# zc402/video-classification

Measured on AMD Instinct MI355X. Metric: clips/sec SlowFast-R50 8x8, 32x224^2 bf16 training step, higher is better.
Workload: dtype bf16

## Files before the change

video-classification_amd/csrc/conv_pw.hip:

```cpp
#include "sfk_common.h"

namespace {

struct PwK {
  const void* x;
  void* y;
  const void* w;
  const void* res;
  const float *scale, *shift, *rscale, *rshift;
  uint8_t* bits;
  const uint8_t* mbits;
  float* parts;
  int xld, xoff, yld, yoff, rld, roff;
  int M, K, cout, relu;
  uint32_t xbytes, ybytes, rbytes;
};

__device__ __forceinline__ int slab_off(int r, int s) { return r * 64 + ((s ^ ((4 - ((r >> 2) & 3)) & 3)) << 4); }

__device__ __forceinline__ void swap16f(float& a, float& b) {
  const auto r = __builtin_amdgcn_permlane16_swap(__float_as_uint(a), __float_as_uint(b), false, false);
  a = __uint_as_float(r[0]);
  b = __uint_as_float(r[1]);
}

template <int NF, int KS, int CG, int NT, bool XDB, int MODE = 0>
__global__ __launch_bounds__(NT, 2) void conv_pw_fused_kernel(const PwK k) {
  constexpr bool DG = MODE == 1;
  constexpr int CW = NF * 16;
  extern __shared__ __attribute__((aligned(16))) char smem[];
  char* wl = smem;
  float* coef = reinterpret_cast<float*>(smem + KS * k.cout * 64);
  const int tid = threadIdx.x, lane = tid & 63, wave = tid >> 6;
  const int l15 = lane & 15, g = lane >> 4;
  {
    const __amdgpu_buffer_rsrc_t wrs = sfk_make_rsrc(k.w, (uint32_t)k.cout * (uint32_t)k.K * 2u);
    const int segs = k.cout * KS * 4;
    for (int i = tid; i < segs; i += NT) {
      const int s = i & 3, ks = (i >> 2) % KS, r = i / (4 * KS);
      const int kk = ks * 32 + s * 8;
      const uint4 v = sfk_buffer_load16(wrs, kk < k.K ? (uint32_t)((r * k.K + kk) * 2) : SFK_OOB);
      *reinterpret_cast<uint4*>(wl + ks * k.cout * 64 + slab_off(r, s)) = v;
    }
    if (MODE == 0) for (int i = tid; i < k.cout; i += NT) {
      coef[i] = k.scale ? k.scale[i] : 1.f;
      coef[k.cout + i] = (k.shift ? k.shift[i] : 0.f) + ((k.res && k.rshift) ? k.rshift[i] : 0.f);
      coef[2 * k.cout + i] = (k.res && k.rscale) ? k.rscale[i] : 1.f;
    }
  }
  __syncthreads();

  const __amdgpu_buffer_rsrc_t xrs = sfk_make_rsrc(k.x, k.xbytes);
  const __amdgpu_buffer_rsrc_t rrs = sfk_make_rsrc(k.res, k.res ? k.rbytes : 0u);
  const bool has_res = k.res != nullptr;
  constexpr int WPB = NT / 64;
  const int wg = (blockIdx.x * WPB + wave);
  const int cgi = wg % CG, wi = wg / CG, nw = (gridDim.x * WPB) / CG;
  const int co_w = cgi * CW;
  const int ntiles = (k.M + 15) >> 4;
  const bf16_t* __restrict__ dummy = nullptr;
  (void)dummy;

  uint4 xc[KS], xn[XDB ? KS : 1];
  uint4 rc[NF / 2], rn[NF / 2];
  uint32_t mc[DG ? NF / 2 : 1], mn[DG ? NF / 2 : 1];
  float csum[DG ? NF / 2 : 1][8];
  if constexpr (DG) {
#pragma unroll
    for (int p = 0; p < NF / 2; ++p)
#pragma unroll
      for (int e = 0; e < 8; ++e) csum[p][e] = 0.f;
  }
  auto issue_x = [&](int tile, uint4 (&xv)[KS]) __attribute__((always_inline)) {
    int m = tile * 16 + l15;
    if (m >= k.M) m = k.M - 1;
    const uint32_t xrow = (uint32_t)(((int64_t)m * k.xld + k.xoff) * 2);
#pragma unroll
    for (int ks = 0; ks < KS; ++ks) {
      const int kk = ks * 32 + g * 8;
      xv[ks] = sfk_buffer_load16(xrs, kk < k.K ? xrow + (uint32_t)(kk * 2) : SFK_OOB);
    }
  };
  auto issue_r = [&](int tile, uint4 (&rv)[NF / 2], uint32_t (&mv)[DG ? NF / 2 : 1]) __attribute__((always_inline)) {
    if (has_res) {
      int m = tile * 16 + l15;
      if (m >= k.M) m = k.M - 1;
      const uint32_t rrow = (uint32_t)(((int64_t)m * k.rld + k.roff + co_w) * 2);
#pragma unroll
      for (int p = 0; p < NF / 2; ++p)
        rv[p] = sfk_buffer_load16(rrs, rrow + (uint32_t)((32 * p + 16 * (g & 1) + 8 * (g >> 1)) * 2));
      if constexpr (DG) {
#pragma unroll
        for (int p = 0; p < NF / 2; ++p)
          mv[p] = k.mbits[(int64_t)m * (k.cout >> 3) + ((co_w + 32 * p + 16 * (g & 1) + 8 * (g >> 1)) >> 3)];
      }
    }
  };

  int tile = wi;
  if (MODE == 0 && tile >= ntiles) return;
  if (tile < ntiles) {
    issue_x(tile, xc);
    issue_r(tile, rc, mc);
  }
  bf16_t* __restrict__ yp = static_cast<bf16_t*>(k.y);
  for (; tile < ntiles; tile += nw) {
    const int nxt = tile + nw;
    if (nxt < ntiles) {
      if constexpr (XDB) issue_x(nxt, reinterpret_cast<uint4(&)[KS]>(xn));
      issue_r(nxt, rn, mn);
    }
    f32x4 acc[NF];
#pragma unroll
    for (int i = 0; i < NF; ++i) acc[i] = f32x4{0.f, 0.f, 0.f, 0.f};
    const char* wlt = wl;
    if constexpr (NF * KS >= 32) asm volatile("" : "+v"(wlt));
#pragma unroll
    for (int ks = 0; ks < KS; ++ks) {
      const bf16x8 b = __builtin_bit_cast(bf16x8, xc[ks]);
#pragma unroll
      for (int i = 0; i < NF; ++i) {
        const bf16x8 a = *reinterpret_cast<const bf16x8*>(wlt + ks * k.cout * 64 + slab_off(co_w + 16 * i + l15, g));
        acc[i] = __builtin_amdgcn_mfma_f32_16x16x32_bf16(a, b, acc[i], 0, 0, 0);
      }
    }
    if constexpr (!XDB) {
      if (nxt < ntiles) issue_x(nxt, xc);
    }
    const int m = tile * 16 + l15;
    const bool rok = m < k.M;
    const int64_t yrow = (int64_t)m * k.yld + k.yoff;
#pragma unroll
    for (int p = 0; p < NF / 2; ++p) {
      float v[8] = {acc[2 * p][0], acc[2 * p][1], acc[2 * p][2], acc[2 * p][3],
                    acc[2 * p + 1][0], acc[2 * p + 1][1], acc[2 * p + 1][2], acc[2 * p + 1][3]};
#pragma unroll
      for (int e = 0; e < 4; ++e) swap16f(v[e], v[4 + e]);
      const int co = co_w + 32 * p + 16 * (g & 1) + 8 * (g >> 1);
      if constexpr (DG) {
        const bf16x8 r8 = __builtin_bit_cast(bf16x8, rc[p]);
        bf16x8 o;
#pragma unroll
        for (int e = 0; e < 8; ++e) {
          const float f = ((mc[p] >> e) & 1u) ? v[e] + (float)r8[e] : 0.f;
          o[e] = (bf16_t)f;
          if (rok) csum[p][e] += (float)o[e];
        }
        if (rok) *reinterpret_cast<bf16x8*>(yp + yrow + co) = o;
        continue;
      }
      const float4 s0 = *reinterpret_cast<const float4*>(coef + co), s1 = *reinterpret_cast<const float4*>(coef + co + 4);
      const float4 h0 = *reinterpret_cast<const float4*>(coef + k.cout + co), h1 = *reinterpret_cast<const float4*>(coef + k.cout + co + 4);
      const float sc[8] = {s0.x, s0.y, s0.z, s0.w, s1.x, s1.y, s1.z, s1.w};
      const float sh[8] = {h0.x, h0.y, h0.z, h0.w, h1.x, h1.y, h1.z, h1.w};
      float f[8];
#pragma unroll
      for (int e = 0; e < 8; ++e) f[e] = v[e] * sc[e] + sh[e];
      if (has_res) {
        const float4 q0 = *reinterpret_cast<const float4*>(coef + 2 * k.cout + co), q1 = *reinterpret_cast<const float4*>(coef + 2 * k.cout + co + 4);
        const float rs[8] = {q0.x, q0.y, q0.z, q0.w, q1.x, q1.y, q1.z, q1.w};
        const bf16x8 r8 = __builtin_bit_cast(bf16x8, rc[p]);
#pragma unroll
        for (int e = 0; e < 8; ++e) f[e] += (float)r8[e] * rs[e];
      }
      uint32_t bits = 0;
      bf16x8 o;
#pragma unroll
      for (int e = 0; e < 8; ++e) {
        if (k.relu) {
          bits |= (f[e] > 0.f ? 1u : 0u) << e;
          f[e] = f[e] > 0.f ? f[e] : 0.f;
        }
        o[e] = (bf16_t)f[e];
      }
      if (rok) {
        *reinterpret_cast<bf16x8*>(yp + yrow + co) = o;
        if (k.bits) k.bits[(int64_t)m * (k.cout >> 3) + (co >> 3)] = (uint8_t)bits;
      }
    }
    if constexpr (XDB) {
#pragma unroll
      for (int ks = 0; ks < KS; ++ks) xc[ks] = xn[ks];
    }
#pragma unroll
    for (int p = 0; p < NF / 2; ++p) rc[p] = rn[p];
    if constexpr (DG) {
#pragma unroll
      for (int p = 0; p < NF / 2; ++p) mc[p] = mn[p];
    }
  }
  if constexpr (DG) {
    float* row = k.parts + (int64_t)wi * k.cout * 2;
#pragma unroll
    for (int p = 0; p < NF / 2; ++p) {
#pragma unroll
      for (int e = 0; e < 8; ++e) {
        float t = csum[p][e];
#pragma unroll
        for (int sft = 1; sft < 16; sft <<= 1) t += __shfl_xor(t, sft);
        csum[p][e] = t;
      }
      if (l15 == 0) {
        const int co = co_w + 32 * p + 16 * (g & 1) + 8 * (g >> 1);
#pragma unroll
        for (int e = 0; e < 8; ++e) *reinterpret_cast<float2*>(row + (co + e) * 2) = make_float2(csum[p][e], 0.f);
      }
    }
  }
}

inline int pw_blocks(int M, int CG, int NT) {
  const int WPB = NT / 64;
  const int ntiles = (M + 15) / 16;
  int blocks = 256 * (NT == 512 ? 1 : 2);
  while ((blocks * WPB) % CG) --blocks;
  int need = (ntiles * CG + WPB - 1) / WPB;
  while ((need * WPB) % CG) ++need;
  return blocks < need ? blocks : need;
}

template <int NF, int KS, int CG, int NT, bool XDB, int MODE = 0>
int pw_launch(const PwK& k, hipStream_t s, int* dry, int kernel) {
  if (dry) {
    *dry = SFK_IGEMM_ROUTE(kernel, 1, 32 * KS, NF * 16 * CG, MODE, 0, 1);
    return SFK_OK;
  }
  const size_t lds = (size_t)KS * k.cout * 64 + (size_t)3 * k.cout * 4;
  static bool attr_set = false;
  if (lds > 64 * 1024 && !attr_set) {
    if (hipFuncSetAttribute(reinterpret_cast<const void*>(&conv_pw_fused_kernel<NF, KS, CG, NT, XDB, MODE>),
                            hipFuncAttributeMaxDynamicSharedMemorySize, (int)lds) != hipSuccess)
      return SFK_ERR_LAUNCH;
    attr_set = true;
  }
  hipLaunchKernelGGL((conv_pw_fused_kernel<NF, KS, CG, NT, XDB, MODE>), dim3(pw_blocks(k.M, CG, NT)), dim3(NT), lds, s, k);
  SFK_CHECK_LAUNCH();
  return SFK_OK;
}

typedef __bf16 bf16x2_t __attribute__((ext_vector_type(2)));

template <int C1, int C2, int CO>
__global__ __launch_bounds__(256, 4) void pw_dual_kernel(const bf16_t* __restrict__ x1, int ld1, int off1,
                                                      const bf16_t* __restrict__ x2, int ld2, int off2,
                                                      const bf16_t* __restrict__ w1, const bf16_t* __restrict__ w2,
                                                      const float* __restrict__ bias, bf16_t* __restrict__ y, int ldy, int offy,
                                                      int64_t pixels) {
  constexpr int KP = (C1 + C2) / 2;
  __shared__ __attribute__((aligned(16))) uint32_t wl[CO * KP];
  __shared__ float bl[CO];
  for (int i = threadIdx.x; i < CO * KP; i += 256) {
    const int co = i / KP, kp = i % KP;
    const bf16_t* src = kp < C1 / 2 ? w1 + co * C1 + 2 * kp : w2 + co * C2 + 2 * (kp - C1 / 2);
    wl[i] = *reinterpret_cast<const uint32_t*>(src);
  }
  if (threadIdx.x < CO) bl[threadIdx.x] = bias ? bias[threadIdx.x] : 0.f;
  __syncthreads();
  constexpr int U = 1;
  for (int64_t p0 = (int64_t)blockIdx.x * 256 * U + threadIdx.x; p0 < pixels; p0 += (int64_t)gridDim.x * 256 * U) {
    uint4 a[U][C1 / 8], b[U][C2 / 8];
#pragma unroll
    for (int u = 0; u < U; ++u) {
      const int64_t p = p0 + u * 256 < pixels ? p0 + u * 256 : p0;
#pragma unroll
      for (int i = 0; i < C1 / 8; ++i) a[u][i] = *reinterpret_cast<const uint4*>(x1 + p * ld1 + off1 + 8 * i);
#pragma unroll
      for (int i = 0; i < C2 / 8; ++i) b[u][i] = *reinterpret_cast<const uint4*>(x2 + p * ld2 + off2 + 8 * i);
    }
    uint32_t woff = 0;
    for (int c8 = 0; c8 < CO; c8 += 8) {
      float acc[U][8];
#pragma unroll
      for (int j = 0; j < 8; ++j) {
        const int co = c8 + j;
#pragma unroll
        for (int u = 0; u < U; ++u) acc[u][j] = bl[co];
#pragma unroll
        for (int q = 0; q < KP / 4; ++q) {
          const uint4 wv = *reinterpret_cast<const uint4*>(&wl[co * KP + 4 * q + woff]);
          const uint32_t wp[4] = {wv.x, wv.y, wv.z, wv.w};
#pragma unroll
          for (int u = 0; u < U; ++u) {
            const uint4 xv = q < C1 / 8 ? a[u][q < C1 / 8 ? q : 0] : b[u][q >= C1 / 8 ? q - C1 / 8 : 0];
            const uint32_t xp[4] = {xv.x, xv.y, xv.z, xv.w};
#pragma unroll
            for (int e = 0; e < 4; ++e)
              acc[u][j] = __builtin_amdgcn_fdot2_f32_bf16(__builtin_bit_cast(bf16x2_t, xp[e]), __builtin_bit_cast(bf16x2_t, wp[e]),
                                                          acc[u][j], false);
          }
        }
        asm volatile("" : "+v"(woff) : "v"(acc[0][j]));
      }
#pragma unroll
      for (int u = 0; u < U; ++u) {
        const int64_t p = p0 + u * 256;
        if (p < pixels) {
          bf16x8 o;
#pragma unroll
          for (int e = 0; e < 8; ++e) o[e] = (bf16_t)acc[u][e];
          *reinterpret_cast<bf16x8*>(y + p * ldy + offy + c8) = o;
        }
      }
    }
  }
}

inline bool pw_dual_map_ok(const sfk_fmap* f) {
  return sfk_fmap_ok(f) && f->dtype == SFK_BF16 && (f->c % 8) == 0 && (f->ld % 8) == 0 && (f->c_off % 8) == 0 &&
         (((uintptr_t)f->ptr) & 15) == 0;
}

}

int sfk_conv_pw_fused(const sfk_conv_desc* d, hipStream_t s, int* dry, int kernel) {
  const sfk_conv_epilogue& e = d->ep;
  const int K = d->cin, C = d->cout;
  if (K > 128 || (K % 8) != 0) return SFK_ERR_UNSUPPORTED;
  if (sfk_fmap_bytes(&d->y) >= (1ll << 32) - 64 || sfk_fmap_bytes(&d->x) >= (1ll << 32) - 64) return SFK_ERR_UNSUPPORTED;
  const int KS = (K + 31) / 32;
  PwK k;
  k.x = d->x.ptr; k.y = d->y.ptr; k.w = d->w; k.res = e.res.ptr;
  k.scale = e.scale; k.shift = e.shift; k.rscale = e.res_scale; k.rshift = e.res_shift;
  k.bits = e.relu_bits; k.mbits = nullptr; k.parts = nullptr;
  k.xld = d->x.ld; k.xoff = d->x.c_off; k.yld = d->y.ld; k.yoff = d->y.c_off;
  k.rld = e.res.ptr ? e.res.ld : 0; k.roff = e.res.ptr ? e.res.c_off : 0;
  k.M = (int)sfk_fmap_pixels(&d->y); k.K = K; k.cout = C; k.relu = e.relu;
  k.xbytes = (uint32_t)sfk_fmap_bytes(&d->x); k.ybytes = (uint32_t)sfk_fmap_bytes(&d->y);
  k.rbytes = e.res.ptr ? (uint32_t)sfk_fmap_bytes(&e.res) : 0u;
  if (d->accumulate) {
    if (k.res) return SFK_ERR_UNSUPPORTED;
    k.res = d->y.ptr; k.rld = d->y.ld; k.roff = d->y.c_off; k.rbytes = k.ybytes;
  }
  if (C == 64 && KS == 2) return pw_launch<4, 2, 1, 256, true>(k, s, dry, kernel);
  if (C == 128 && KS == 4) return pw_launch<8, 4, 1, 256, true>(k, s, dry, kernel);
  if (C == 32 && KS == 1) return pw_launch<2, 1, 1, 256, true>(k, s, dry, kernel);
  if (C == 64 && KS == 1) return pw_launch<4, 1, 1, 256, true>(k, s, dry, kernel);
  if (C == 128 && KS == 1) return pw_launch<8, 1, 1, 256, true>(k, s, dry, kernel);
  if (C == 256 && KS == 2) return sfk_tune().igemm_pw_stream == 2 ? pw_launch<4, 2, 4, 256, true>(k, s, dry, kernel) : pw_launch<8, 2, 2, 256, true>(k, s, dry, kernel);
  if (C == 512 && KS == 4) return pw_launch<4, 4, 8, 512, true>(k, s, dry, kernel);
  if (C == 320 && KS == 4 && !k.res) return pw_launch<4, 4, 5, 512, true>(k, s, dry, kernel);
  return SFK_ERR_UNSUPPORTED;
}

int sfk_conv_pw_dgrad_rows(const sfk_conv_desc* d) {
  if (sfk_fmap_bytes(&d->y) >= (1ll << 32) - 64 || sfk_fmap_bytes(&d->x) >= (1ll << 32) - 64) return 0;
  const int M = (int)sfk_fmap_pixels(&d->y);
  if (d->cin == 64 && d->cout == 256) return pw_blocks(M, 2, 256) * 4 / 2;
  if (d->cin == 128 && d->cout == 512) return pw_blocks(M, 8, 512) * 8 / 8;
  return 0;
}

int sfk_conv_pw_dgrad(const sfk_conv_desc* d, hipStream_t s, int* dry) {
  PwK k;
  k.x = d->x.ptr; k.y = d->y.ptr; k.w = d->w; k.res = d->y.ptr;
  k.scale = k.shift = k.rscale = k.rshift = nullptr;
  k.bits = nullptr; k.mbits = d->out_relu_bits; k.parts = d->bnb.partials;
  k.xld = d->x.ld; k.xoff = d->x.c_off; k.yld = d->y.ld; k.yoff = d->y.c_off; k.rld = d->y.ld; k.roff = d->y.c_off;
  k.M = (int)sfk_fmap_pixels(&d->y); k.K = d->cin; k.cout = d->cout; k.relu = 0;
  k.xbytes = (uint32_t)sfk_fmap_bytes(&d->x); k.ybytes = (uint32_t)sfk_fmap_bytes(&d->y); k.rbytes = k.ybytes;
  if (d->cin == 64 && d->cout == 256) return pw_launch<8, 2, 2, 256, true, 1>(k, s, dry, SFK_IK_PWD);
  if (d->cin == 128 && d->cout == 512) return pw_launch<4, 4, 8, 512, true, 1>(k, s, dry, SFK_IK_PWD);
  return SFK_ERR_UNSUPPORTED;
}

extern "C" int sfk_conv_pw_dual_supported(const sfk_fmap* x1, const sfk_fmap* x2, const sfk_fmap* y) {
  if (!x1 || !x2 || !y || !pw_dual_map_ok(x1) || !pw_dual_map_ok(x2) || !pw_dual_map_ok(y)) return 0;
  if (sfk_fmap_pixels(x1) != sfk_fmap_pixels(y) || sfk_fmap_pixels(x2) != sfk_fmap_pixels(y)) return 0;
  return (x1->c == 32 && x2->c == 8 && y->c == 8) || (x1->c == 64 && x2->c == 16 && y->c == 16);
}

extern "C" int sfk_conv_pw_dual(const sfk_fmap* x1, const void* w1, const sfk_fmap* x2, const void* w2, const float* bias,
                                const sfk_fmap* y, sfk_stream_t stream) {
  if (!x1 || !x2 || !y || !w1 || !w2 || !sfk_fmap_ok(x1) || !sfk_fmap_ok(x2) || !sfk_fmap_ok(y)) return SFK_ERR_INVALID;
  if (!sfk_conv_pw_dual_supported(x1, x2, y)) return SFK_ERR_UNSUPPORTED;
  if ((((uintptr_t)w1) | ((uintptr_t)w2)) & 3) return SFK_ERR_INVALID;
  const int64_t px = sfk_fmap_pixels(y);
  int64_t blocks = (px + 255) / 256;
  if (blocks > 4096) blocks = 4096;
  hipStream_t s = static_cast<hipStream_t>(stream);
  const bf16_t *a = static_cast<const bf16_t*>(x1->ptr), *b = static_cast<const bf16_t*>(x2->ptr);
  const bf16_t *u = static_cast<const bf16_t*>(w1), *v = static_cast<const bf16_t*>(w2);
  bf16_t* o = static_cast<bf16_t*>(y->ptr);
  if (y->c == 8)
    hipLaunchKernelGGL((pw_dual_kernel<32, 8, 8>), dim3((unsigned)blocks), dim3(256), 0, s, a, x1->ld, x1->c_off, b, x2->ld, x2->c_off,
                       u, v, bias, o, y->ld, y->c_off, px);
  else
    hipLaunchKernelGGL((pw_dual_kernel<64, 16, 16>), dim3((unsigned)blocks), dim3(256), 0, s, a, x1->ld, x1->c_off, b, x2->ld, x2->c_off,
                       u, v, bias, o, y->ld, y->c_off, px);
  SFK_CHECK_LAUNCH();
  return SFK_OK;
}
```

Measured before the change: 1176.

## Add wide pointwise conv kernel with deeper prefetch for 512/320-channel outputs

Adds a new pointwise-conv forward kernel for the C=512 and C=320 (K=128) cases. Each wave computes a wider strip of output channels, NF=8 or 10 instead of 4, reading filter fragments from LDS per tile rather than keeping them in registers. It also keeps two tiles of input and residual loads in flight ahead of compute. The aim is to cut redundant activation reads across channel groups and to hide global-load latency. The cost is higher register pressure and repeated LDS filter reads. The old path stays reachable through a tuning flag bit.

```diff
diff --git a/video-classification_amd/csrc/conv_pw.hip b/video-classification_amd/csrc/conv_pw.hip
--- a/video-classification_amd/csrc/conv_pw.hip
+++ b/video-classification_amd/csrc/conv_pw.hip
@@ -209,6 +209,136 @@
   }
 }
 
+template <int NF, int KS>
+__device__ __forceinline__ void pw_wide_tile(const PwK& k, const char* wl, const float* coef, const int tile, const int co_w,
+                                             const int l15, const int g, const bool has_res, const uint4 (&xc)[KS],
+                                             const uint4 (&rc)[NF / 2]) {
+  f32x4 acc[NF];
+#pragma unroll
+  for (int i = 0; i < NF; ++i) acc[i] = f32x4{0.f, 0.f, 0.f, 0.f};
+  int wo = 0;
+  asm volatile("" : "+v"(wo));
+  const char* wlt = wl + wo;
+#pragma unroll
+  for (int ks = 0; ks < KS; ++ks) {
+    const bf16x8 b = __builtin_bit_cast(bf16x8, xc[ks]);
+#pragma unroll
+    for (int i = 0; i < NF; ++i) {
+      const bf16x8 a = *reinterpret_cast<const bf16x8*>(wlt + ks * k.cout * 64 + slab_off(co_w + 16 * i + l15, g));
+      acc[i] = __builtin_amdgcn_mfma_f32_16x16x32_bf16(a, b, acc[i], 0, 0, 0);
+    }
+  }
+  bf16_t* __restrict__ yp = static_cast<bf16_t*>(k.y);
+  const int m = tile * 16 + l15;
+  const bool rok = m < k.M;
+  const int64_t yrow = (int64_t)m * k.yld + k.yoff;
+#pragma unroll
+  for (int p = 0; p < NF / 2; ++p) {
+    float v[8] = {acc[2 * p][0], acc[2 * p][1], acc[2 * p][2], acc[2 * p][3],
+                  acc[2 * p + 1][0], acc[2 * p + 1][1], acc[2 * p + 1][2], acc[2 * p + 1][3]};
+#pragma unroll
+    for (int e = 0; e < 4; ++e) swap16f(v[e], v[4 + e]);
+    const int co = co_w + 32 * p + 16 * (g & 1) + 8 * (g >> 1);
+    const float4 s0 = *reinterpret_cast<const float4*>(coef + co), s1 = *reinterpret_cast<const float4*>(coef + co + 4);
+    const float4 h0 = *reinterpret_cast<const float4*>(coef + k.cout + co), h1 = *reinterpret_cast<const float4*>(coef + k.cout + co + 4);
+    const float sc[8] = {s0.x, s0.y, s0.z, s0.w, s1.x, s1.y, s1.z, s1.w};
+    const float sh[8] = {h0.x, h0.y, h0.z, h0.w, h1.x, h1.y, h1.z, h1.w};
+    float f[8];
+#pragma unroll
+    for (int e = 0; e < 8; ++e) f[e] = v[e] * sc[e] + sh[e];
+    uint4 rr = rc[p];
+    asm volatile("" : "+v"(rr.x), "+v"(rr.y), "+v"(rr.z), "+v"(rr.w));
+    if (has_res) {
+      const float4 q0 = *reinterpret_cast<const float4*>(coef + 2 * k.cout + co), q1 = *reinterpret_cast<const float4*>(coef + 2 * k.cout + co + 4);
+      const float rs[8] = {q0.x, q0.y, q0.z, q0.w, q1.x, q1.y, q1.z, q1.w};
+      const bf16x8 r8 = __builtin_bit_cast(bf16x8, rr);
+#pragma unroll
+      for (int e = 0; e < 8; ++e) f[e] += (float)r8[e] * rs[e];
+    }
+    uint32_t bits = 0;
+    bf16x8 o;
+#pragma unroll
+    for (int e = 0; e < 8; ++e) {
+      if (k.relu) {
+        bits |= (f[e] > 0.f ? 1u : 0u) << e;
+        f[e] = f[e] > 0.f ? f[e] : 0.f;
+      }
+      o[e] = (bf16_t)f[e];
+    }
+    if (rok) {
+      *reinterpret_cast<bf16x8*>(yp + yrow + co) = o;
+      if (k.bits) k.bits[(int64_t)m * (k.cout >> 3) + (co >> 3)] = (uint8_t)bits;
+    }
+  }
+}
+
+template <int NF, int KS, int CG, int NT, int PD>
+__global__ __launch_bounds__(NT, 2) void conv_pw_wide_kernel(const PwK k) {
+  static_assert(NF * KS >= 32, "pw_wide_tile re-reads the filter fragments: fewer of them belong in registers (kernel above)");
+  constexpr int CW = NF * 16, NS = PD + 1, WPB = NT / 64;
+  extern __shared__ __attribute__((aligned(16))) char smem[];
+  char* wl = smem;
+  float* coef = reinterpret_cast<float*>(smem + KS * k.cout * 64);
+  const int tid = threadIdx.x, lane = tid & 63, wave = __builtin_amdgcn_readfirstlane(tid >> 6);
+  const int l15 = lane & 15, g = lane >> 4;
+  {
+    const __amdgpu_buffer_rsrc_t wrs = sfk_make_rsrc(k.w, (uint32_t)k.cout * (uint32_t)k.K * 2u);
+    const int segs = k.cout * KS * 4;
+    for (int i = tid; i < segs; i += NT) {
+      const int s = i & 3, ks = (i >> 2) % KS, r = i / (4 * KS);
+      const int kk = ks * 32 + s * 8;
+      const uint4 v = sfk_buffer_load16(wrs, kk < k.K ? (uint32_t)((r * k.K + kk) * 2) : SFK_OOB);
+      *reinterpret_cast<uint4*>(wl + ks * k.cout * 64 + slab_off(r, s)) = v;
+    }
+    for (int i = tid; i < k.cout; i += NT) {
+      coef[i] = k.scale ? k.scale[i] : 1.f;
+      coef[k.cout + i] = (k.shift ? k.shift[i] : 0.f) + ((k.res && k.rshift) ? k.rshift[i] : 0.f);
+      coef[2 * k.cout + i] = (k.res && k.rscale) ? k.rscale[i] : 1.f;
+    }
+  }
+  __syncthreads();
+
+  const __amdgpu_buffer_rsrc_t xrs = sfk_make_rsrc(k.x, k.xbytes);
+  const __amdgpu_buffer_rsrc_t rrs = sfk_make_rsrc(k.res, k.res ? k.rbytes : 0u);
+  const bool has_res = k.res != nullptr;
+  const int wg = (blockIdx.x * WPB + wave);
+  const int cgi = wg % CG, wi = wg / CG, nw = (gridDim.x * WPB) / CG;
+  const int co_w = cgi * CW;
+  const int ntiles = (k.M + 15) >> 4;
+
+  uint4 xq[NS][KS], rq[NS][NF / 2];
+  auto issue = [&](int tile, uint4 (&xv)[KS], uint4 (&rv)[NF / 2]) __attribute__((always_inline)) {
+    const bool live = tile < ntiles;
+    int m = tile * 16 + l15;
+    if (m >= k.M) m = k.M - 1;
+    const uint32_t xrow = (uint32_t)(((int64_t)m * k.xld + k.xoff) * 2);
+#pragma unroll
+    for (int ks = 0; ks < KS; ++ks) {
+      const int kk = ks * 32 + g * 8;
+      xv[ks] = sfk_buffer_load16(xrs, (live && kk < k.K) ? xrow + (uint32_t)(kk * 2) : SFK_OOB);
+    }
+    const uint32_t rrow = (uint32_t)(((int64_t)m * k.rld + k.roff + co_w) * 2);
+#pragma unroll
+    for (int p = 0; p < NF / 2; ++p)
+      rv[p] = sfk_buffer_load16(rrs, (live && has_res) ? rrow + (uint32_t)((32 * p + 16 * (g & 1) + 8 * (g >> 1)) * 2) : SFK_OOB);
+  };
+
+#pragma unroll
+  for (int u = 0; u < PD; ++u) {
+    issue(wi + u * nw, xq[u], rq[u]);
+    __builtin_amdgcn_sched_barrier(0);
+  }
+  const int mine = wi < ntiles ? (ntiles - wi + nw - 1) / nw : 0;
+  const int rounds = (mine + NS - 1) / NS;
+  for (int r = 0, tile = wi; r < rounds; ++r) {
+#pragma unroll
+    for (int u = 0; u < NS; ++u, tile += nw) {
+      issue(tile + PD * nw, xq[(u + PD) % NS], rq[(u + PD) % NS]);
+      pw_wide_tile<NF, KS>(k, wl, coef, tile, co_w, l15, g, has_res, xq[u], rq[u]);
+    }
+  }
+}
+
 inline int pw_blocks(int M, int CG, int NT) {
   const int WPB = NT / 64;
   const int ntiles = (M + 15) / 16;
@@ -234,6 +364,25 @@
     attr_set = true;
   }
   hipLaunchKernelGGL((conv_pw_fused_kernel<NF, KS, CG, NT, XDB, MODE>), dim3(pw_blocks(k.M, CG, NT)), dim3(NT), lds, s, k);
+  SFK_CHECK_LAUNCH();
+  return SFK_OK;
+}
+
+template <int NF, int KS, int CG, int NT, int PD>
+int pw_launch_wide(const PwK& k, hipStream_t s, int* dry, int kernel) {
+  if (dry) {
+    *dry = SFK_IGEMM_ROUTE(kernel, 1, 32 * KS, NF * 16 * CG, 0, 0, 1);
+    return SFK_OK;
+  }
+  const size_t lds = (size_t)KS * k.cout * 64 + (size_t)3 * k.cout * 4;
+  static bool attr_set = false;
+  if (lds > 64 * 1024 && !attr_set) {
+    if (hipFuncSetAttribute(reinterpret_cast<const void*>(&conv_pw_wide_kernel<NF, KS, CG, NT, PD>),
+                            hipFuncAttributeMaxDynamicSharedMemorySize, (int)lds) != hipSuccess)
+      return SFK_ERR_LAUNCH;
+    attr_set = true;
+  }
+  hipLaunchKernelGGL((conv_pw_wide_kernel<NF, KS, CG, NT, PD>), dim3(pw_blocks(k.M, CG, NT)), dim3(NT), lds, s, k);
   SFK_CHECK_LAUNCH();
   return SFK_OK;
 }
@@ -337,8 +486,9 @@
   if (C == 64 && KS == 1) return pw_launch<4, 1, 1, 256, true>(k, s, dry, kernel);
   if (C == 128 && KS == 1) return pw_launch<8, 1, 1, 256, true>(k, s, dry, kernel);
   if (C == 256 && KS == 2) return sfk_tune().igemm_pw_stream == 2 ? pw_launch<4, 2, 4, 256, true>(k, s, dry, kernel) : pw_launch<8, 2, 2, 256, true>(k, s, dry, kernel);
-  if (C == 512 && KS == 4) return pw_launch<4, 4, 8, 512, true>(k, s, dry, kernel);
-  if (C == 320 && KS == 4 && !k.res) return pw_launch<4, 4, 5, 512, true>(k, s, dry, kernel);
+  const bool prev = (sfk_tune().igemm_pw_stream & 16) != 0;
+  if (C == 512 && KS == 4) return prev ? pw_launch<4, 4, 8, 512, true>(k, s, dry, kernel) : pw_launch_wide<8, 4, 4, 512, 2>(k, s, dry, kernel);
+  if (C == 320 && KS == 4 && !k.res) return prev ? pw_launch<4, 4, 5, 512, true>(k, s, dry, kernel) : pw_launch_wide<10, 4, 2, 512, 2>(k, s, dry, kernel);
   return SFK_ERR_UNSUPPORTED;
 }
 
```

After: 1181 (median of 6 runs). About the same (+0.4%).
